# arrufat/zignal

Hardware: NVIDIA H100
Metric: Mpixels/sec Gaussian-blur 8K RGBA f32 (higher is better)
Workload: dtype f32

## Files before the change

zignal_b200/csrc/zb_conv_fused.cu:

```cuda
#include "zb_conv.h"
#include "zb_device.cuh"
#include "zb_shard.h"
#include "zb_tma.cuh"

namespace zb {

namespace {

constexpr int TW = 256;
constexpr int CHUNK = 8;
constexpr int G = TW / 8 + 2;
constexpr int STAGE_BYTES = G * CHUNK * 128;
constexpr int RING_ROWS = 24;
constexpr int RING_ROW_BYTES = TW * 16;
constexpr int RING_BYTES = RING_ROWS * RING_ROW_BYTES;
constexpr int NTHREADS = 256;
constexpr int MAX_HALF = 8;
constexpr int MAXK = 2 * MAX_HALF + 1;
constexpr int smem_bytes(int stages) { return stages * STAGE_BYTES + RING_BYTES + 64 + 1024; }

struct FusedParams {
    float kx[MAXK];
    float ky[MAXK];
    const float4* src;
    float4* dst;
    unsigned long long src_pitch_px, dst_pitch_px;
    int rows, cols, border;
    int ngroups;
    int n_strips, n_bands, band_rows;
    int row0, row1;
    int fix_rows;
    int fix_left;
    int fix_right;
    int tma_row_off;
    int edge_fast;
    int lsrc[8];
    int rsrc[8];
};

struct ShardParams {
    const float4* up_rows;
    const float4* down_rows;
    unsigned long long up_pitch_px, down_pitch_px;
    int half;
    ShardLink link;
};

template <bool EXACT>
__device__ __forceinline__ void mac4(float4& acc, const float4& v, float k) {
    if constexpr (EXACT) {
        acc.x = __fadd_rn(acc.x, __fmul_rn(v.x, k));
        acc.y = __fadd_rn(acc.y, __fmul_rn(v.y, k));
        acc.z = __fadd_rn(acc.z, __fmul_rn(v.z, k));
        acc.w = __fadd_rn(acc.w, __fmul_rn(v.w, k));
    } else {
        acc.x = fmaf(v.x, k, acc.x);
        acc.y = fmaf(v.y, k, acc.y);
        acc.z = fmaf(v.z, k, acc.z);
        acc.w = fmaf(v.w, k, acc.w);
    }
}

template <int NT, bool SHARD = false>
__device__ __noinline__ void fixup_stage(uint32_t stage, int y0, int xs0, bool fix_x, bool fix_rows, const FusedParams& p,
                                         int nb_lo = 0, int nb_hi = 0) {
    const int xlimit = p.ngroups * 8;
    auto stage_addr = [&](int rr, int xx) {
        const uint32_t line = (uint32_t)(rr * G + (xx >> 3));
        return stage + line * 128 + ((((uint32_t)xx & 7u) ^ (line & 7u)) << 4);
    };
    if (fix_x && p.edge_fast) {
        fix_x = false;
        if (threadIdx.x < 128) {
            const int side = threadIdx.x >> 6, rr = (threadIdx.x >> 3) & 7, e = threadIdx.x & 7;
            const int y = y0 + rr;
            bool row_ok = y >= 0 && y < p.rows;
            if constexpr (SHARD) row_ok = row_ok || (y < 0 && y >= nb_lo) || (y >= p.rows && y < nb_hi);
            const bool edge = side == 0 ? xs0 < 0 : xs0 + G * 8 > p.cols;
            if (row_ok && edge) {
                const int s_dst = side == 0 ? e : p.cols - xs0 + e;
                const int s_src = side == 0 ? p.lsrc[e] : p.rsrc[e] - xs0;
                if (s_dst < G * 8) sts128(stage_addr(rr, s_dst), lds128(stage_addr(rr, s_src)));
            }
        }
    }
    if (fix_x) {
        const int nleft = xs0 < 0 ? min(-xs0, G * 8) : 0;
        const int r0 = max(0, xlimit - xs0);
        const int r1 = min(G * 8, p.cols - xs0 + MAX_HALF);
        const int per_row = nleft + max(0, r1 - r0);
        for (int idx = threadIdx.x; idx < CHUNK * per_row; idx += NT) {
            const int rr = idx / per_row, e = idx - rr * per_row;
            const int xx = e < nleft ? e : r0 + (e - nleft);
            const int y = y0 + rr, x = xs0 + xx;
            const float4* rowp = p.src + (long long)y * (long long)p.src_pitch_px;
            if (y < 0 || y >= p.rows) {
                if constexpr (SHARD) {
                    if (y < nb_lo || y >= nb_hi) continue;
                } else {
                    continue;
                }
            }
            const int rx = resolve_index(x, p.cols, p.border);
            float4 v = make_float4(0.f, 0.f, 0.f, 0.f);
            if (rx >= 0) {
                const int sx = rx - xs0;
                if (rx < xlimit && sx >= 0 && sx < G * 8) v = lds128(stage_addr(rr, sx));
                else v = __ldg(rowp + rx);
            }
            sts128(stage_addr(rr, xx), v);
        }
    }
    if (fix_rows) {
        for (int idx = threadIdx.x; idx < CHUNK * G * 8; idx += NT) {
            const int rr = idx / (G * 8);
            const int xx = idx - rr * (G * 8);
            const int y = y0 + rr, x = xs0 + xx;
            if (y >= 0 && y < p.rows) continue;
            if constexpr (SHARD) {
                if (y >= nb_lo && y < nb_hi) continue;
            }
            const int ry = resolve_index(y, p.rows, p.border);
            const int rx = resolve_index(x, p.cols, p.border);
            float4 v = make_float4(0.f, 0.f, 0.f, 0.f);
            if (ry >= 0 && rx >= 0) v = __ldg(p.src + (size_t)ry * p.src_pitch_px + rx);
            sts128(stage_addr(rr, xx), v);
        }
    }
}

template <int HALF, bool EXACT, int SLOT>
__device__ __forceinline__ void v_pass(uint32_t v_col, const FusedParams& p, float4* out, bool col_ok, int rows_left) {
    constexpr int K = 2 * HALF + 1;
    constexpr int NLOAD = CHUNK + 2 * HALF;
    float4 acc[8];
#pragma unroll
    for (int o = 0; o < 8; ++o) acc[o] = make_float4(0.f, 0.f, 0.f, 0.f);
#pragma unroll
    for (int j = 0; j < NLOAD; ++j) {
        const int sr = (SLOT * CHUNK + 8 - HALF + j) % RING_ROWS;
        const float4 v = lds128(v_col + (uint32_t)(sr * RING_ROW_BYTES));
#pragma unroll
        for (int o = 0; o < 8; ++o) {
            const int ti = j - o;
            if (ti >= 0 && ti < K) mac4<EXACT>(acc[o], v, p.ky[ti]);
        }
    }
    if (col_ok) {
#pragma unroll
        for (int o = 0; o < 8; ++o)
            if (o < rows_left) __stcs(out + (size_t)o * p.dst_pitch_px, acc[o]);
    }
}

template <int HALF, bool EXACT, int STAGES, bool SHARD>
__device__ __forceinline__ uint32_t fused_units(const CUtensorMap& tmap, const FusedParams& p, unsigned nbr, int k_begin, int k_end, uint32_t count0) {
    constexpr int K = 2 * HALF + 1;
    constexpr int NLOAD = CHUNK + 2 * HALF;
    extern __shared__ unsigned char smem_raw[];
    const uint32_t smem0 = (smem_u32(smem_raw) + 1023u) & ~1023u;
    const uint32_t ring = smem0 + STAGES * STAGE_BYTES;
    const uint32_t bar0 = ring + RING_BYTES;

    const int tid = threadIdx.x;
    const long long u_first = (long long)blockIdx.x + (long long)k_begin * gridDim.x;
    const long long u_last = (long long)blockIdx.x + (long long)k_end * gridDim.x;
    const int n_units = (int)min((long long)p.n_strips * p.n_bands, u_last);
    if (u_first >= n_units) return count0;
    auto touches_neighbour = [&](int y) { return ((nbr & 1u) && y < 0) || ((nbr & 2u) && y + CHUNK > p.rows); };

    int pu = (int)u_first, pi = 0;
    uint32_t pcount = count0;
    auto produce = [&]() {
        if (pu >= n_units) return;
        int band = pu / p.n_strips;
        const int strip = pu - band * p.n_strips;
        if constexpr (SHARD) band = band + 1 == p.n_bands ? 0 : band + 1;
        const int ra = p.row0 + band * p.band_rows;
        const int rb = min(ra + p.band_rows, p.row1);
        const int n_in = (rb - ra + CHUNK - 1) / CHUNK + 2;
        const uint32_t st = pcount % STAGES;
        const int y = ra - CHUNK + CHUNK * pi;
        fence_proxy_async();
        mbar_arrive_expect_tx(bar0 + 8 * st, STAGE_BYTES);
        tma_load_3d(smem0 + st * STAGE_BYTES, &tmap, 0, strip * (TW / 8) - 1, y + p.tma_row_off, bar0 + 8 * st);
        ++pcount;
        if (++pi == n_in) { pi = 0; pu += gridDim.x; }
    };
    if (tid == 0)
        for (int i = 0; i < STAGES; ++i) produce();

    const int ht = tid & 31, hr = tid >> 5;
    const int vx = tid;
    const uint32_t v_col = ring + (uint32_t)(vx >> 3) * 128u + ((((uint32_t)vx & 7u) ^ (((uint32_t)vx >> 3) & 7u)) << 4);
    const uint32_t h_ring_col = ring + (uint32_t)ht * 128u;
    const uint32_t h_key = (uint32_t)ht & 7u;

    uint32_t ccount = count0;

    for (int unit = (int)u_first; unit < n_units; unit += gridDim.x) {
        int band = unit / p.n_strips;
        const int strip = unit - band * p.n_strips;
        if constexpr (SHARD) band = band + 1 == p.n_bands ? 0 : band + 1;
        const int x0 = strip * TW;
        const int ra = p.row0 + band * p.band_rows;
        const int rb = min(ra + p.band_rows, p.row1);
        const int n_out = (rb - ra + CHUNK - 1) / CHUNK;
        const int n_in = n_out + 2;
        const int g0 = x0 / 8 - 1;

        for (int i = 0; i < n_in; ++i, ++ccount) {
            const uint32_t st = ccount % STAGES;
            const uint32_t stage = smem0 + st * STAGE_BYTES;
            while (!mbar_try_wait(bar0 + 8 * st, (ccount / STAGES) & 1u)) {}
            const int y0 = ra - CHUNK + CHUNK * i;
            bool fix_r = p.fix_rows && (y0 < 0 || y0 + CHUNK > p.rows);
            if constexpr (SHARD) {
                if (touches_neighbour(y0)) fix_r = false;
            }
            const bool fix_x = (p.fix_left && g0 < 0) || (p.fix_right && (g0 + G) * 8 > p.ngroups * 8);
            if (fix_r || fix_x) {
                fixup_stage<NTHREADS, SHARD>(stage, y0, g0 * 8, fix_x, fix_r, p, (nbr & 1u) ? INT_MIN : 0, (nbr & 2u) ? INT_MAX : p.rows);
                __syncthreads();
            }

            {
                const uint32_t line0 = (uint32_t)(hr * G + ht);
                uint32_t lbase[3];
#pragma unroll
                for (int l = 0; l < 3; ++l) lbase[l] = stage + (line0 + l) * 128u + (((line0 + l) & 7u) << 4);
                const uint32_t rrow = h_ring_col + (uint32_t)(((i % 3) * CHUNK + hr) * RING_ROW_BYTES);
                float4 acc[8];
#pragma unroll
                for (int o = 0; o < 8; ++o) acc[o] = make_float4(0.f, 0.f, 0.f, 0.f);
#pragma unroll
                for (int j = 0; j < NLOAD; ++j) {
                    const int pidx = 8 - HALF + j;
                    const float4 v = lds128(lbase[pidx >> 3] ^ (((uint32_t)pidx & 7u) << 4));
#pragma unroll
                    for (int o = 0; o < 8; ++o) {
                        const int ti = j - o;
                        if (ti >= 0 && ti < K) mac4<EXACT>(acc[o], v, p.kx[ti]);
                    }
                }
#pragma unroll
                for (int o = 0; o < 8; ++o) sts128(rrow + ((((uint32_t)o) ^ h_key) << 4), acc[o]);
            }
            __syncthreads();

            if (tid == 0) produce();

            if (i >= 2) {
                const int c = i - 2;
                const int x = x0 + vx;
                const int yb = ra + CHUNK * c;
                float4* out = p.dst + (size_t)yb * p.dst_pitch_px + x;
                const bool col_ok = x < p.cols;
                switch (c % 3) {
                    case 0: v_pass<HALF, EXACT, 0>(v_col, p, out, col_ok, rb - yb); break;
                    case 1: v_pass<HALF, EXACT, 1>(v_col, p, out, col_ok, rb - yb); break;
                    default: v_pass<HALF, EXACT, 2>(v_col, p, out, col_ok, rb - yb); break;
                }
            }
            __syncthreads();
        }
    }
    return ccount;
}

template <int HALF, bool EXACT, int STAGES>
__device__ __forceinline__ uint32_t fused_units_call(const CUtensorMap& tmap, const FusedParams& p, unsigned nbr, int k_begin, int k_end, uint32_t count0) {
    return fused_units<HALF, EXACT, STAGES, true>(tmap, p, nbr, k_begin, k_end, count0);
}

template <int HALF, bool EXACT, int STAGES, bool SHARD>
__device__ __forceinline__ void fused_sep_rgbaf32_body(const CUtensorMap& tmap, const FusedParams& p, const ShardParams* sp) {
    extern __shared__ unsigned char smem_raw[];
    const uint32_t smem0 = (smem_u32(smem_raw) + 1023u) & ~1023u;
    const uint32_t bar0 = smem0 + STAGES * STAGE_BYTES + RING_BYTES;
    const int tid = threadIdx.x;
    if (tid == 0) {
        asm volatile("prefetch.tensormap [%0];" ::"l"(&tmap) : "memory");
        for (int i = 0; i < STAGES; ++i) mbar_init(bar0 + 8 * i, 1);
        fence_barrier_init();
    }
    if constexpr (!SHARD) {
        __syncthreads();
        fused_units<HALF, EXACT, STAGES, false>(tmap, p, 0u, 0, INT_MAX / 2048, 0u);
    } else {
        ShardCtrl* me = sp->link.self;
        const unsigned long long epoch = sp->link.epoch;
        const unsigned nbr = (sp->up_rows ? 1u : 0u) | (sp->down_rows ? 2u : 0u);
        const int per_side = sp->half * p.cols;
        const int total = (sp->up_rows ? per_side : 0) + (sp->down_rows ? per_side : 0);
        constexpr int BATCH = 12;
        const int rem = (p.n_strips * p.n_bands) % (int)gridDim.x;
        const int n_copiers = (int)gridDim.x - rem;
        const int ci = (int)blockIdx.x - rem;
        const bool copier = ci >= 0 && (long long)ci * NTHREADS * BATCH < total;
        if (tid == 0) {
            if (blockIdx.x == 0) {
                me->dbg[0] = global_timer_ns();
                if (sp->link.up) st_release_sys(&sp->link.up->ready_from[1], epoch);
                if (sp->link.down) st_release_sys(&sp->link.down->ready_from[0], epoch);
            }
            if (copier) {
                if (sp->up_rows) shard_wait_ge(&me->ready_from[0], epoch, me);
                if (sp->down_rows) shard_wait_ge(&me->ready_from[1], epoch, me);
                if (ci == 0) me->dbg[1] = global_timer_ns();
            }
        }
        __syncthreads();
        if (copier) {
            for (int base = ci * NTHREADS * BATCH; base < total; base += n_copiers * NTHREADS * BATCH) {
                float4 v[BATCH];
                float4* dstp[BATCH];
    #pragma unroll
                for (int k = 0; k < BATCH; ++k) {
                    int e = base + k * NTHREADS + tid;
                    dstp[k] = nullptr;
                    if (e < total) {
                        const bool upper = sp->up_rows && e < per_side;
                        if (!upper && sp->up_rows) e -= per_side;
                        const int r = e / p.cols, x = e - r * p.cols;
                        if (upper) {
                            v[k] = *(sp->up_rows + (size_t)r * sp->up_pitch_px + x);
                            dstp[k] = const_cast<float4*>(p.src) + (long long)(r - sp->half) * (long long)p.src_pitch_px + x;
                        } else {
                            v[k] = *(sp->down_rows + (size_t)r * sp->down_pitch_px + x);
                            dstp[k] = const_cast<float4*>(p.src) + (long long)(p.rows + r) * (long long)p.src_pitch_px + x;
                        }
                    }
                }
    #pragma unroll
                for (int k = 0; k < BATCH; ++k)
                    if (dstp[k]) *dstp[k] = v[k];
            }
            asm volatile("fence.proxy.async;" ::: "memory");
            __syncthreads();
        }
        if (tid == 0) {
            __threadfence();
            if (atomicAdd(&me->halo_reads[0], 1u) == gridDim.x - 1u) {
                me->halo_reads[0] = 0;
                me->dbg[2] = global_timer_ns();
                __threadfence();
                st_release_sys(&me->halo_landed, epoch);
                if (sp->up_rows) st_release_sys(&sp->link.up->done_from[1], epoch);
                if (sp->down_rows) st_release_sys(&sp->link.down->done_from[0], epoch);
            }
        }
        const long long first_halo_unit = (long long)max(0, p.n_bands - 2) * p.n_strips;
        const int k_split = first_halo_unit <= (long long)blockIdx.x ? 0 : (int)((first_halo_unit - blockIdx.x + gridDim.x - 1) / gridDim.x);
        const uint32_t count = fused_units_call<HALF, EXACT, STAGES>(tmap, p, nbr, 0, k_split, 0u);
        if ((long long)blockIdx.x + (long long)k_split * gridDim.x < (long long)p.n_strips * p.n_bands) {
            if (tid == 0) {
                shard_wait_ge(&me->halo_landed, epoch, me);
                asm volatile("fence.proxy.async;" ::: "memory");
            }
            __syncthreads();
            fused_units_call<HALF, EXACT, STAGES>(tmap, p, nbr, k_split, INT_MAX / 2048, count);
        }
        if (tid == 0) {
            ShardCtrl* me = sp->link.self;
            __threadfence();
            if (atomicAdd(&me->exit_ticket, 1u) == gridDim.x - 1u) {
                me->exit_ticket = 0;
                me->dbg[3] = global_timer_ns();
                if (sp->link.up) shard_wait_ge(&me->done_from[0], sp->link.epoch, me);
                if (sp->link.down) shard_wait_ge(&me->done_from[1], sp->link.epoch, me);
                me->dbg[4] = global_timer_ns();
            }
        }
    }
}


template <int HALF, bool EXACT, int STAGES>
__global__ void __launch_bounds__(NTHREADS, 1)
fused_sep_rgbaf32_kernel(const __grid_constant__ CUtensorMap tmap, const __grid_constant__ FusedParams p) {
    fused_sep_rgbaf32_body<HALF, EXACT, STAGES, false>(tmap, p, nullptr);
}

template <int HALF, bool EXACT, int STAGES>
__global__ void __launch_bounds__(NTHREADS, 1)
fused_sep_rgbaf32_shard_kernel(const __grid_constant__ CUtensorMap tmap, const __grid_constant__ FusedParams p,
                               const __grid_constant__ ShardParams sp) {
    fused_sep_rgbaf32_body<HALF, EXACT, STAGES, true>(tmap, p, &sp);
}

template <int HALF, bool EXACT, int STAGES>
int launch_one(const CUtensorMap& tmap, const FusedParams& p, int grid, cudaStream_t s) {
    auto k = fused_sep_rgbaf32_kernel<HALF, EXACT, STAGES>;
    ZB_CUDA(cudaFuncSetAttribute(k, cudaFuncAttributeMaxDynamicSharedMemorySize, smem_bytes(STAGES)));
    k<<<grid, NTHREADS, smem_bytes(STAGES), s>>>(tmap, p);
    ZB_LAUNCHED();
    return ZB_OK;
}


constexpr int WS_RING_ROWS = 32;
constexpr int WS_RING_BYTES = WS_RING_ROWS * RING_ROW_BYTES;
constexpr int WS_THREADS = 544;
constexpr int WS_SMEM_BYTES = 2 * STAGE_BYTES + WS_RING_BYTES + 128 + 1024;

__device__ __forceinline__ void mbar_arrive(uint32_t bar) {
    asm volatile("mbarrier.arrive.shared::cta.b64 _, [%0];" ::"r"(bar) : "memory");
}
__device__ __forceinline__ void mbar_wait(uint32_t bar, uint32_t parity) {
    while (!mbar_try_wait(bar, parity)) {}
}
__device__ __forceinline__ void named_bar_sync(int id, int nthreads) {
    asm volatile("bar.sync %0, %1;" ::"r"(id), "r"(nthreads) : "memory");
}

struct UnitGeom {
    int x0, ra, rb, n_out, n_in, g0;
};
__device__ __forceinline__ UnitGeom unit_geom(int unit, const FusedParams& p) {
    UnitGeom u;
    const int band = unit / p.n_strips, strip = unit - band * p.n_strips;
    u.x0 = strip * TW;
    u.ra = p.row0 + band * p.band_rows;
    u.rb = min(u.ra + p.band_rows, p.row1);
    u.n_out = (u.rb - u.ra + CHUNK - 1) / CHUNK;
    u.n_in = u.n_out + 2;
    u.g0 = u.x0 / 8 - 1;
    return u;
}

template <int HALF, bool EXACT>
__global__ void __launch_bounds__(WS_THREADS, 1)
fused_sep_rgbaf32_ws_kernel(const __grid_constant__ CUtensorMap tmap, const __grid_constant__ FusedParams p) {
    constexpr int K = 2 * HALF + 1;
    constexpr int NLOAD = CHUNK + 2 * HALF;
    extern __shared__ unsigned char smem_raw[];
    const uint32_t smem0 = (smem_u32(smem_raw) + 1023u) & ~1023u;
    const uint32_t ring = smem0 + 2 * STAGE_BYTES;
    const uint32_t bars = ring + WS_RING_BYTES;
    const uint32_t full_stage = bars, empty_stage = bars + 16, full_ring = bars + 32, empty_ring = bars + 64;

    const int tid = threadIdx.x;
    const int n_units = p.n_strips * p.n_bands;
    if (tid == 0) {
        for (int i = 0; i < 2; ++i) { mbar_init(full_stage + 8 * i, 1); mbar_init(empty_stage + 8 * i, 256); }
        for (int i = 0; i < 4; ++i) { mbar_init(full_ring + 8 * i, 256); mbar_init(empty_ring + 8 * i, 256); }
        fence_barrier_init();
    }
    __syncthreads();

    if (tid >= 512) {
        if (tid == 512) {
            asm volatile("prefetch.tensormap [%0];" ::"l"(&tmap) : "memory");
            uint32_t g = 0;
            for (int unit = blockIdx.x; unit < n_units; unit += gridDim.x) {
                const UnitGeom u = unit_geom(unit, p);
                for (int i = 0; i < u.n_in; ++i, ++g) {
                    const uint32_t st = g & 1u;
                    if (g >= 2) mbar_wait(empty_stage + 8 * st, ((g >> 1) - 1) & 1u);
                    fence_proxy_async();
                    mbar_arrive_expect_tx(full_stage + 8 * st, STAGE_BYTES);
                    tma_load_3d(smem0 + st * STAGE_BYTES, &tmap, 0, u.g0, u.ra - CHUNK + CHUNK * i, full_stage + 8 * st);
                }
            }
        }
    } else if (tid < 256) {
        const int ht = tid & 31, hr = tid >> 5;
        const uint32_t h_key = (uint32_t)ht & 7u;
        uint32_t g = 0;
        for (int unit = blockIdx.x; unit < n_units; unit += gridDim.x) {
            const UnitGeom u = unit_geom(unit, p);
            for (int i = 0; i < u.n_in; ++i, ++g) {
                const uint32_t st = g & 1u, slot = g & 3u;
                const uint32_t stage = smem0 + st * STAGE_BYTES;
                mbar_wait(full_stage + 8 * st, (g >> 1) & 1u);
                const int y0 = u.ra - CHUNK + CHUNK * i;
                const bool fix_r = p.fix_rows && (y0 < 0 || y0 + CHUNK > p.rows);
                const bool fix_x = (p.fix_left && u.g0 < 0) || (p.fix_right && (u.g0 + G) * 8 > p.ngroups * 8);
                if (fix_r || fix_x) {
                    fixup_stage<256>(stage, y0, u.g0 * 8, fix_x, fix_r, p);
                    named_bar_sync(1, 256);
                }
                float4 acc[8];
#pragma unroll
                for (int o = 0; o < 8; ++o) acc[o] = make_float4(0.f, 0.f, 0.f, 0.f);
                const uint32_t line0 = (uint32_t)(hr * G + ht);
                uint32_t lbase[3];
#pragma unroll
                for (int l = 0; l < 3; ++l) lbase[l] = stage + (line0 + l) * 128u + (((line0 + l) & 7u) << 4);
#pragma unroll
                for (int j = 0; j < NLOAD; ++j) {
                    const int pidx = 8 - HALF + j;
                    const float4 v = lds128(lbase[pidx >> 3] ^ (((uint32_t)pidx & 7u) << 4));
#pragma unroll
                    for (int o = 0; o < 8; ++o) {
                        const int ti = j - o;
                        if (ti >= 0 && ti < K) mac4<EXACT>(acc[o], v, p.kx[ti]);
                    }
                }
                mbar_arrive(empty_stage + 8 * st);
                if (g >= 4) mbar_wait(empty_ring + 8 * slot, ((g >> 2) - 1) & 1u);
                const uint32_t rrow = ring + (uint32_t)ht * 128u + (uint32_t)((slot * CHUNK + hr) * RING_ROW_BYTES);
#pragma unroll
                for (int o = 0; o < 8; ++o) sts128(rrow + ((((uint32_t)o) ^ h_key) << 4), acc[o]);
                mbar_arrive(full_ring + 8 * slot);
            }
        }
    } else {
        const int vx = tid - 256;
        const uint32_t v_col = ring + (uint32_t)(vx >> 3) * 128u + ((((uint32_t)vx & 7u) ^ (((uint32_t)vx >> 3) & 7u)) << 4);
        const uint32_t ring_end = v_col + WS_RING_BYTES;
        uint32_t gbase = 0;
        for (int unit = blockIdx.x; unit < n_units; unit += gridDim.x) {
            const UnitGeom u = unit_geom(unit, p);
            for (int c = 0; c < u.n_out; ++c) {
                const uint32_t gl = gbase + c + 2;
                mbar_wait(full_ring + 8 * (gl & 3u), (gl >> 2) & 1u);
                float4 acc[8];
#pragma unroll
                for (int o = 0; o < 8; ++o) acc[o] = make_float4(0.f, 0.f, 0.f, 0.f);
                const uint32_t a0 = v_col + (uint32_t)((((gbase + c) & 3u) * CHUNK + 8 - HALF) * RING_ROW_BYTES);
#pragma unroll
                for (int j = 0; j < NLOAD; ++j) {
                    uint32_t a = a0 + (uint32_t)(j * RING_ROW_BYTES);
                    if (a >= ring_end) a -= WS_RING_BYTES;
                    const float4 v = lds128(a);
#pragma unroll
                    for (int o = 0; o < 8; ++o) {
                        const int ti = j - o;
                        if (ti >= 0 && ti < K) mac4<EXACT>(acc[o], v, p.ky[ti]);
                    }
                }
                mbar_arrive(empty_ring + 8 * ((gbase + c) & 3u));
                if (c == u.n_out - 1) {
                    mbar_arrive(empty_ring + 8 * ((gbase + c + 1) & 3u));
                    mbar_arrive(empty_ring + 8 * ((gbase + c + 2) & 3u));
                }
                const int x = u.x0 + vx;
                const int yb = u.ra + CHUNK * c;
                if (x < p.cols) {
                    float4* out = p.dst + (size_t)yb * p.dst_pitch_px + x;
#pragma unroll
                    for (int o = 0; o < 8; ++o)
                        if (yb + o < u.rb) __stcs(out + (size_t)o * p.dst_pitch_px, acc[o]);
                }
            }
            gbase += (uint32_t)u.n_in;
        }
    }
}

template <int HALF, bool EXACT>
int launch_ws(const CUtensorMap& tmap, const FusedParams& p, int grid, cudaStream_t s) {
    auto k = fused_sep_rgbaf32_ws_kernel<HALF, EXACT>;
    ZB_CUDA(cudaFuncSetAttribute(k, cudaFuncAttributeMaxDynamicSharedMemorySize, WS_SMEM_BYTES));
    k<<<grid, WS_THREADS, WS_SMEM_BYTES, s>>>(tmap, p);
    ZB_LAUNCHED();
    return ZB_OK;
}

template <int HALF>
int launch_fused(const CUtensorMap& tmap, const FusedParams& p, int grid, bool exact, cudaStream_t s) {
    int variant = g_tune_variant.load();
    if (variant < 0) variant = HALF <= 5 ? 1 : 0;
    if (variant == 1) return exact ? launch_ws<HALF, true>(tmap, p, grid, s) : launch_ws<HALF, false>(tmap, p, grid, s);
    if (exact) return launch_one<HALF, true, 2>(tmap, p, grid, s);
    return g_tune_stages.load() == 2 ? launch_one<HALF, false, 2>(tmap, p, grid, s) : launch_one<HALF, false, 3>(tmap, p, grid, s);
}

}

static int encode_block_map(EncodeTiledFn encode, CUtensorMap& tmap, void* data, int ngroups, int rows, uint64_t stride_px) {
    const cuuint64_t gdim[3] = {32, (cuuint64_t)ngroups, (cuuint64_t)rows};
    const cuuint64_t gstr[2] = {128, (cuuint64_t)stride_px * 16};
    const cuuint32_t box[3] = {32, (cuuint32_t)G, (cuuint32_t)CHUNK};
    const cuuint32_t estr[3] = {1, 1, 1};
    CUresult cr = encode(&tmap, CU_TENSOR_MAP_DATA_TYPE_FLOAT32, 3, data, gdim, gstr, box, estr, CU_TENSOR_MAP_INTERLEAVE_NONE,
                         CU_TENSOR_MAP_SWIZZLE_128B, CU_TENSOR_MAP_L2_PROMOTION_L2_256B, CU_TENSOR_MAP_FLOAT_OOB_FILL_NONE);
    if (cr != CUDA_SUCCESS) {
        snprintf(t_last_error, sizeof(t_last_error), "cuTensorMapEncodeTiled failed: %d", (int)cr);
        return ZB_ERR_UNSUPPORTED;
    }
    return ZB_OK;
}

static int fused_prepare(const zb_image* src, zb_image* dst, const float* kx, int nx, const float* ky, int ny, int border, int row0, int row1,
                         FusedParams& p, CUtensorMap& tmap, int& grid, int& half_out, EncodeTiledFn& encode) {
    const int half_x = nx / 2, half_y = ny / 2;
    const int half = half_x > half_y ? half_x : half_y;
    if (half < 1 || half > MAX_HALF) return ZB_ERR_UNSUPPORTED;
    if (src->cols < 16 || src->rows < 16) return ZB_ERR_UNSUPPORTED;
    if (images_overlap(src, dst, 16)) return ZB_ERR_UNSUPPORTED;
    if (((uintptr_t)src->data & 15u) || ((uintptr_t)dst->data & 15u)) return ZB_ERR_UNSUPPORTED;
    for (int i = 0; i < nx; ++i) if (fabsf(kx[i]) < 1e-10f) return ZB_ERR_UNSUPPORTED;
    for (int i = 0; i < ny; ++i) if (fabsf(ky[i]) < 1e-10f) return ZB_ERR_UNSUPPORTED;
    encode = encode_tiled_fn();
    if (!encode) return ZB_ERR_UNSUPPORTED;
    DeviceInfo di;
    int rc = device_info(&di);
    if (rc) return rc;
    if (di.smem_optin < (size_t)smem_bytes(3)) return ZB_ERR_UNSUPPORTED;

    memset(&p, 0, sizeof(p));
    for (int i = 0; i < nx; ++i) p.kx[i + (half - half_x)] = kx[i];
    for (int i = 0; i < ny; ++i) p.ky[i + (half - half_y)] = ky[i];
    p.src = (const float4*)src->data;
    p.dst = (float4*)dst->data;
    p.src_pitch_px = src->stride;
    p.dst_pitch_px = dst->stride;
    p.rows = (int)src->rows;
    p.cols = (int)src->cols;
    p.border = border;
    p.ngroups = p.cols / 8;
    p.n_strips = (p.cols + TW - 1) / TW;
    p.row0 = row0 < 0 ? 0 : row0;
    p.row1 = (row1 < 0 || row1 > p.rows) ? p.rows : row1;
    if (p.row1 <= p.row0) { grid = 0; return ZB_OK; }
    const int nrows = p.row1 - p.row0;
    const int band_target = g_tune_band_rows.load();
    int n_bands = (nrows + band_target - 1) / band_target;
    const long long waves = ((long long)n_bands * p.n_strips + di.sm_count - 1) / di.sm_count;
    int nb2 = (int)((waves * di.sm_count) / p.n_strips);
    if (nb2 > n_bands) n_bands = nb2;
    int band_rows = (nrows + n_bands - 1) / n_bands;
    band_rows = ((band_rows + CHUNK - 1) / CHUNK) * CHUNK;
    if (band_rows < 64) band_rows = 64;
    p.band_rows = band_rows;
    p.n_bands = (nrows + band_rows - 1) / band_rows;
    p.fix_rows = border != ZB_BORDER_ZERO;
    p.fix_left = border != ZB_BORDER_ZERO;
    p.fix_right = (border != ZB_BORDER_ZERO) || (p.cols % 8 != 0);
    p.edge_fast = g_tune_edge_fast.load() && (border == ZB_BORDER_REPLICATE || border == ZB_BORDER_MIRROR) && p.cols % 8 == 0 && p.cols >= 16;
    for (int e = 0; e < 8; ++e) {
        const int xl = e - 8, xr = p.cols + e;
        p.lsrc[e] = 8 + (border == ZB_BORDER_REPLICATE ? 0 : -xl);
        p.rsrc[e] = border == ZB_BORDER_REPLICATE ? p.cols - 1 : 2 * (p.cols - 1) - xr;
    }

    if ((rc = encode_block_map(encode, tmap, src->data, p.ngroups, p.rows, src->stride))) return rc;
    const int n_units = p.n_strips * p.n_bands;
    grid = n_units < di.sm_count ? n_units : di.sm_count;
    half_out = half;
    return ZB_OK;
}

int conv_separable_fused_rgbaf32(const zb_image* src, zb_image* dst, const float* kx, int nx, const float* ky, int ny, int border,
                                 bool exact, cudaStream_t s, int row0, int row1) {
    FusedParams p;
    CUtensorMap tmap;
    EncodeTiledFn encode;
    int grid = 0, half = 0;
    int rc = fused_prepare(src, dst, kx, nx, ky, ny, border, row0, row1, p, tmap, grid, half, encode);
    if (rc || grid == 0) return rc;
    t_last_kernel = exact ? "fused_sep_rgbaf32_exact" : "fused_sep_rgbaf32";
    switch (half) {
        case 1: return launch_fused<1>(tmap, p, grid, exact, s);
        case 2: return launch_fused<2>(tmap, p, grid, exact, s);
        case 3: return launch_fused<3>(tmap, p, grid, exact, s);
        case 4: return launch_fused<4>(tmap, p, grid, exact, s);
        case 5: return launch_fused<5>(tmap, p, grid, exact, s);
        case 6: return launch_fused<6>(tmap, p, grid, exact, s);
        case 7: return launch_fused<7>(tmap, p, grid, exact, s);
        case 8: return launch_fused<8>(tmap, p, grid, exact, s);
    }
    return ZB_ERR_UNSUPPORTED;
}

template <int HALF>
static int launch_shard(const CUtensorMap& tmap, const FusedParams& p, const ShardParams& sp,
                        int grid, bool exact, cudaStream_t s) {
    if (exact) {
        auto k = fused_sep_rgbaf32_shard_kernel<HALF, true, 2>;
        ZB_CUDA(cudaFuncSetAttribute(k, cudaFuncAttributeMaxDynamicSharedMemorySize, smem_bytes(2)));
        k<<<grid, NTHREADS, smem_bytes(2), s>>>(tmap, p, sp);
    } else if (g_tune_stages.load() == 3) {
        auto k = fused_sep_rgbaf32_shard_kernel<HALF, false, 3>;
        ZB_CUDA(cudaFuncSetAttribute(k, cudaFuncAttributeMaxDynamicSharedMemorySize, smem_bytes(3)));
        k<<<grid, NTHREADS, smem_bytes(3), s>>>(tmap, p, sp);
    } else {
        auto k = fused_sep_rgbaf32_shard_kernel<HALF, false, 2>;
        ZB_CUDA(cudaFuncSetAttribute(k, cudaFuncAttributeMaxDynamicSharedMemorySize, smem_bytes(2)));
        k<<<grid, NTHREADS, smem_bytes(2), s>>>(tmap, p, sp);
    }
    ZB_LAUNCHED();
    return ZB_OK;
}

int conv_separable_fused_rgbaf32_shard(const zb_image* src, zb_image* dst, const float* kx, int nx, const float* ky, int ny, int border,
                                       bool exact, const PeerBlock& up, const PeerBlock& down, uint32_t halo_cap, const ShardLink& link,
                                       cudaStream_t s) {
    if (src->rows % CHUNK != 0 || halo_cap < (uint32_t)CHUNK) return ZB_ERR_UNSUPPORTED;
    FusedParams p;
    CUtensorMap tmap;
    EncodeTiledFn encode;
    int grid = 0, half = 0;
    int rc = fused_prepare(src, dst, kx, nx, ky, ny, border, 0, -1, p, tmap, grid, half, encode);
    if (rc) return rc;
    if (grid == 0) return ZB_ERR_UNSUPPORTED;
    if (p.band_rows % CHUNK != 0) return ZB_ERR_UNSUPPORTED;
    const uint32_t hv = (uint32_t)(ny / 2);
    if ((up.data && (up.rows < hv || ((uintptr_t)up.data & 15u))) || (down.data && (down.rows < hv || ((uintptr_t)down.data & 15u))))
        return ZB_ERR_UNSUPPORTED;
    void* ext = (char*)src->data - (size_t)halo_cap * src->stride * 16;
    if ((rc = encode_block_map(encode, tmap, ext, p.ngroups, (int)(src->rows + 2 * halo_cap), src->stride))) return rc;
    p.tma_row_off = (int)halo_cap;
    p.fix_rows = 1;
    ShardParams sp;
    memset(&sp, 0, sizeof(sp));
    sp.half = (int)hv;
    if (up.data && hv) {
        sp.up_rows = (const float4*)up.data + (size_t)(up.rows - hv) * up.stride;
        sp.up_pitch_px = up.stride;
    }
    if (down.data && hv) {
        sp.down_rows = (const float4*)down.data;
        sp.down_pitch_px = down.stride;
    }
    sp.link = link;
    if (!sp.up_rows) sp.link.up = nullptr;
    if (!sp.down_rows) sp.link.down = nullptr;
    {
        DeviceInfo di;
        if ((rc = device_info(&di))) return rc;
        grid = di.sm_count;
    }
    t_last_kernel = exact ? "fused_sep_rgbaf32_shard_exact" : "fused_sep_rgbaf32_shard";
    switch (half) {
        case 1: return launch_shard<1>(tmap, p, sp, grid, exact, s);
        case 2: return launch_shard<2>(tmap, p, sp, grid, exact, s);
        case 3: return launch_shard<3>(tmap, p, sp, grid, exact, s);
        case 4: return launch_shard<4>(tmap, p, sp, grid, exact, s);
        case 5: return launch_shard<5>(tmap, p, sp, grid, exact, s);
        case 6: return launch_shard<6>(tmap, p, sp, grid, exact, s);
        case 7: return launch_shard<7>(tmap, p, sp, grid, exact, s);
        case 8: return launch_shard<8>(tmap, p, sp, grid, exact, s);
    }
    return ZB_ERR_UNSUPPORTED;
}

}
```

Before: 80270.

## Handle x-edge borders inline in fused h-pass and search band size by step count

Adds an EDGE-templated horizontal pass that remaps out-of-range column loads to replicate or mirror sources in registers, so edge strips no longer run a separate shared-memory fixup stage with an extra barrier when edge_fast is enabled. For the non-warp-specialized variant without x patching, band height is now chosen by an exhaustive search that minimizes waves times chunk steps, including the two halo chunks per band, instead of using a fixed target. The intent is to cut border fixup work and the pipeline fill overhead that comes from poor band sizing. The cost is a second compiled h-pass variant, and very small bands would raise halo overhead.

```diff
diff --git a/zignal_b200/csrc/zb_conv_fused.cu b/zignal_b200/csrc/zb_conv_fused.cu
--- a/zignal_b200/csrc/zb_conv_fused.cu
+++ b/zignal_b200/csrc/zb_conv_fused.cu
@@ -153,10 +153,41 @@
     }
 }
 
+template <int HALF, bool EXACT, bool EDGE>
+__device__ __forceinline__ void h_pass(uint32_t stage, uint32_t rrow, int ht, int hr, const FusedParams& p, bool lthr, bool rthr,
+                                       bool mirror) {
+    constexpr int K = 2 * HALF + 1;
+    constexpr int NLOAD = CHUNK + 2 * HALF;
+    const uint32_t line0 = (uint32_t)(hr * G + ht);
+    uint32_t lbase[3];
+#pragma unroll
+    for (int l = 0; l < 3; ++l) lbase[l] = stage + (line0 + l) * 128u + (((line0 + l) & 7u) << 4);
+    auto pix = [&](int s) { return lbase[s >> 3] ^ (((uint32_t)s & 7u) << 4); };
+    float4 acc[8];
+#pragma unroll
+    for (int o = 0; o < 8; ++o) acc[o] = make_float4(0.f, 0.f, 0.f, 0.f);
+#pragma unroll
+    for (int j = 0; j < NLOAD; ++j) {
+        const int pidx = 8 - HALF + j;
+        uint32_t a = pix(pidx);
+        if constexpr (EDGE) {
+            if (pidx < 8 && lthr) a = mirror ? pix(16 - pidx) : pix(8);
+            if (pidx >= 16 && rthr) a = mirror ? pix(30 - pidx) : pix(15);
+        }
+        const float4 v = lds128(a);
+#pragma unroll
+        for (int o = 0; o < 8; ++o) {
+            const int ti = j - o;
+            if (ti >= 0 && ti < K) mac4<EXACT>(acc[o], v, p.kx[ti]);
+        }
+    }
+    const uint32_t h_key = (uint32_t)ht & 7u;
+#pragma unroll
+    for (int o = 0; o < 8; ++o) sts128(rrow + ((((uint32_t)o) ^ h_key) << 4), acc[o]);
+}
+
 template <int HALF, bool EXACT, int STAGES, bool SHARD>
 __device__ __forceinline__ uint32_t fused_units(const CUtensorMap& tmap, const FusedParams& p, unsigned nbr, int k_begin, int k_end, uint32_t count0) {
-    constexpr int K = 2 * HALF + 1;
-    constexpr int NLOAD = CHUNK + 2 * HALF;
     extern __shared__ unsigned char smem_raw[];
     const uint32_t smem0 = (smem_u32(smem_raw) + 1023u) & ~1023u;
     const uint32_t ring = smem0 + STAGES * STAGE_BYTES;
@@ -194,7 +225,6 @@
     const int vx = tid;
     const uint32_t v_col = ring + (uint32_t)(vx >> 3) * 128u + ((((uint32_t)vx & 7u) ^ (((uint32_t)vx >> 3) & 7u)) << 4);
     const uint32_t h_ring_col = ring + (uint32_t)ht * 128u;
-    const uint32_t h_key = (uint32_t)ht & 7u;
 
     uint32_t ccount = count0;
 
@@ -208,6 +238,12 @@
         const int n_out = (rb - ra + CHUNK - 1) / CHUNK;
         const int n_in = n_out + 2;
         const int g0 = x0 / 8 - 1;
+        const bool x_edge = g0 < 0 || (g0 + G) * 8 > p.ngroups * 8;
+        const bool edge_x = p.edge_fast && x_edge;
+        const bool fix_x = !p.edge_fast && ((p.fix_left && g0 < 0) || (p.fix_right && (g0 + G) * 8 > p.ngroups * 8));
+        const bool lthr = g0 < 0 && ht == 0;
+        const bool rthr = g0 + 1 + ht == p.ngroups - 1;
+        const bool mirror = p.border == ZB_BORDER_MIRROR;
 
         for (int i = 0; i < n_in; ++i, ++ccount) {
             const uint32_t st = ccount % STAGES;
@@ -218,34 +254,14 @@
             if constexpr (SHARD) {
                 if (touches_neighbour(y0)) fix_r = false;
             }
-            const bool fix_x = (p.fix_left && g0 < 0) || (p.fix_right && (g0 + G) * 8 > p.ngroups * 8);
             if (fix_r || fix_x) {
                 fixup_stage<NTHREADS, SHARD>(stage, y0, g0 * 8, fix_x, fix_r, p, (nbr & 1u) ? INT_MIN : 0, (nbr & 2u) ? INT_MAX : p.rows);
                 __syncthreads();
             }
 
-            {
-                const uint32_t line0 = (uint32_t)(hr * G + ht);
-                uint32_t lbase[3];
-#pragma unroll
-                for (int l = 0; l < 3; ++l) lbase[l] = stage + (line0 + l) * 128u + (((line0 + l) & 7u) << 4);
-                const uint32_t rrow = h_ring_col + (uint32_t)(((i % 3) * CHUNK + hr) * RING_ROW_BYTES);
-                float4 acc[8];
-#pragma unroll
-                for (int o = 0; o < 8; ++o) acc[o] = make_float4(0.f, 0.f, 0.f, 0.f);
-#pragma unroll
-                for (int j = 0; j < NLOAD; ++j) {
-                    const int pidx = 8 - HALF + j;
-                    const float4 v = lds128(lbase[pidx >> 3] ^ (((uint32_t)pidx & 7u) << 4));
-#pragma unroll
-                    for (int o = 0; o < 8; ++o) {
-                        const int ti = j - o;
-                        if (ti >= 0 && ti < K) mac4<EXACT>(acc[o], v, p.kx[ti]);
-                    }
-                }
-#pragma unroll
-                for (int o = 0; o < 8; ++o) sts128(rrow + ((((uint32_t)o) ^ h_key) << 4), acc[o]);
-            }
+            const uint32_t rrow = h_ring_col + (uint32_t)(((i % 3) * CHUNK + hr) * RING_ROW_BYTES);
+            if (edge_x) h_pass<HALF, EXACT, true>(stage, rrow, ht, hr, p, lthr, rthr, mirror);
+            else h_pass<HALF, EXACT, false>(stage, rrow, ht, hr, p, false, false, false);
             __syncthreads();
 
             if (tid == 0) produce();
@@ -559,11 +575,14 @@
     return ZB_OK;
 }
 
+int fused_variant(int half) {
+    const int variant = g_tune_variant.load();
+    return variant < 0 ? (half <= 5 ? 1 : 0) : variant;
+}
+
 template <int HALF>
 int launch_fused(const CUtensorMap& tmap, const FusedParams& p, int grid, bool exact, cudaStream_t s) {
-    int variant = g_tune_variant.load();
-    if (variant < 0) variant = HALF <= 5 ? 1 : 0;
-    if (variant == 1) return exact ? launch_ws<HALF, true>(tmap, p, grid, s) : launch_ws<HALF, false>(tmap, p, grid, s);
+    if (fused_variant(HALF) == 1) return exact ? launch_ws<HALF, true>(tmap, p, grid, s) : launch_ws<HALF, false>(tmap, p, grid, s);
     if (exact) return launch_one<HALF, true, 2>(tmap, p, grid, s);
     return g_tune_stages.load() == 2 ? launch_one<HALF, false, 2>(tmap, p, grid, s) : launch_one<HALF, false, 3>(tmap, p, grid, s);
 }
@@ -585,7 +604,7 @@
 }
 
 static int fused_prepare(const zb_image* src, zb_image* dst, const float* kx, int nx, const float* ky, int ny, int border, int row0, int row1,
-                         FusedParams& p, CUtensorMap& tmap, int& grid, int& half_out, EncodeTiledFn& encode) {
+                         bool shard, FusedParams& p, CUtensorMap& tmap, int& grid, int& half_out, EncodeTiledFn& encode) {
     const int half_x = nx / 2, half_y = ny / 2;
     const int half = half_x > half_y ? half_x : half_y;
     if (half < 1 || half > MAX_HALF) return ZB_ERR_UNSUPPORTED;
@@ -613,24 +632,37 @@
     p.border = border;
     p.ngroups = p.cols / 8;
     p.n_strips = (p.cols + TW - 1) / TW;
+    p.fix_rows = border != ZB_BORDER_ZERO;
+    p.fix_left = border != ZB_BORDER_ZERO;
+    p.fix_right = (border != ZB_BORDER_ZERO) || (p.cols % 8 != 0);
+    p.edge_fast = g_tune_edge_fast.load() && (border == ZB_BORDER_REPLICATE || border == ZB_BORDER_MIRROR) && p.cols % 8 == 0 && p.cols >= 16;
     p.row0 = row0 < 0 ? 0 : row0;
     p.row1 = (row1 < 0 || row1 > p.rows) ? p.rows : row1;
     if (p.row1 <= p.row0) { grid = 0; return ZB_OK; }
     const int nrows = p.row1 - p.row0;
-    const int band_target = g_tune_band_rows.load();
-    int n_bands = (nrows + band_target - 1) / band_target;
-    const long long waves = ((long long)n_bands * p.n_strips + di.sm_count - 1) / di.sm_count;
-    int nb2 = (int)((waves * di.sm_count) / p.n_strips);
-    if (nb2 > n_bands) n_bands = nb2;
-    int band_rows = (nrows + n_bands - 1) / n_bands;
-    band_rows = ((band_rows + CHUNK - 1) / CHUNK) * CHUNK;
-    if (band_rows < 64) band_rows = 64;
+    int band_rows;
+    const bool x_patch = (p.fix_left || p.fix_right) && !p.edge_fast;
+    if (!shard && fused_variant(half) == 0 && !x_patch) {
+        long long best = LLONG_MAX;
+        band_rows = CHUNK;
+        for (int n_runs = 1; n_runs <= (nrows + CHUNK - 1) / CHUNK; ++n_runs) {
+            const int run_rows = ((nrows + n_runs - 1) / n_runs + CHUNK - 1) / CHUNK * CHUNK;
+            const long long units = (long long)((nrows + run_rows - 1) / run_rows) * p.n_strips;
+            const long long steps = (units + di.sm_count - 1) / di.sm_count * (run_rows / CHUNK + 2);
+            if (steps < best) { best = steps; band_rows = run_rows; }
+        }
+    } else {
+        const int band_target = g_tune_band_rows.load();
+        int n_bands = (nrows + band_target - 1) / band_target;
+        const long long waves = ((long long)n_bands * p.n_strips + di.sm_count - 1) / di.sm_count;
+        int nb2 = (int)((waves * di.sm_count) / p.n_strips);
+        if (nb2 > n_bands) n_bands = nb2;
+        band_rows = (nrows + n_bands - 1) / n_bands;
+        band_rows = ((band_rows + CHUNK - 1) / CHUNK) * CHUNK;
+        if (band_rows < 64) band_rows = 64;
+    }
     p.band_rows = band_rows;
     p.n_bands = (nrows + band_rows - 1) / band_rows;
-    p.fix_rows = border != ZB_BORDER_ZERO;
-    p.fix_left = border != ZB_BORDER_ZERO;
-    p.fix_right = (border != ZB_BORDER_ZERO) || (p.cols % 8 != 0);
-    p.edge_fast = g_tune_edge_fast.load() && (border == ZB_BORDER_REPLICATE || border == ZB_BORDER_MIRROR) && p.cols % 8 == 0 && p.cols >= 16;
     for (int e = 0; e < 8; ++e) {
         const int xl = e - 8, xr = p.cols + e;
         p.lsrc[e] = 8 + (border == ZB_BORDER_REPLICATE ? 0 : -xl);
@@ -650,7 +682,7 @@
     CUtensorMap tmap;
     EncodeTiledFn encode;
     int grid = 0, half = 0;
-    int rc = fused_prepare(src, dst, kx, nx, ky, ny, border, row0, row1, p, tmap, grid, half, encode);
+    int rc = fused_prepare(src, dst, kx, nx, ky, ny, border, row0, row1, false, p, tmap, grid, half, encode);
     if (rc || grid == 0) return rc;
     t_last_kernel = exact ? "fused_sep_rgbaf32_exact" : "fused_sep_rgbaf32";
     switch (half) {
@@ -694,7 +726,7 @@
     CUtensorMap tmap;
     EncodeTiledFn encode;
     int grid = 0, half = 0;
-    int rc = fused_prepare(src, dst, kx, nx, ky, ny, border, 0, -1, p, tmap, grid, half, encode);
+    int rc = fused_prepare(src, dst, kx, nx, ky, ny, border, 0, -1, true, p, tmap, grid, half, encode);
     if (rc) return rc;
     if (grid == 0) return ZB_ERR_UNSUPPORTED;
     if (p.band_rows % CHUNK != 0) return ZB_ERR_UNSUPPORTED;
```

After: 84390, median of 6. +5.1%, better.
